# rcelha/rio-rs

Hardware: AMD Instinct MI355X
Metric: placement decisions/sec + achieved HBM GB/s, 10M objects x 1 024 nodes (higher is better)
Workload: dtype u32; 1 GPU; config 3: 10000000 objects x 1024 nodes, Zipf(1.1) load, cap 1.25x; a stream of committed ticks that starts from the cold table (all pending); objects_per_gpu=10000000, nodes=1024, parallelism=rows sharded x1

## Files before the change

### include/rio_gpu_placement_debug.h

```cpp
#ifndef RIO_GPU_PLACEMENT_DEBUG_H
#define RIO_GPU_PLACEMENT_DEBUG_H

#include "rio_gpu_placement.h"

#ifdef __cplusplus
extern "C" {
#endif

int rio_gp_debug_set_compact(rio_gp_t* h, int mode);
uint64_t rio_gp_debug_chained_scans(rio_gp_t* h);
int rio_gp_debug_set_speculate(rio_gp_t* h, int speculate);
int rio_gp_debug_set_node_index(rio_gp_t* h, uint32_t tile_rows);
int rio_gp_debug_node_index_geometry(rio_gp_t* h, const uint64_t* node_bitmap, uint32_t* out4);
void rio_gp_debug_set_scan_nt(int mode);
void rio_gp_debug_set_part_shift(int shift);
uint64_t rio_gp_debug_wave_row_lo(uint64_t n_objects, uint32_t n_nodes, uint32_t wave, uint32_t* n_waves);
int rio_gp_debug_ktrace(rio_gp_t* h, int enable, int table, uint64_t* out2048);
int rio_gp_debug_stream_probe(rio_gp_t* h, int mode, int reps, float* ms);

#ifdef __cplusplus
}
#endif
#endif
```

### rio-rs_amd/csrc/placement_kernels.h

```cpp
#pragma once
#include <hip/hip_runtime.h>
#include <stdint.h>

namespace riogp {

typedef uint32_t u32;
typedef unsigned long long u64;

constexpr u32 kNone = 0xFFFFFFFFu;
constexpr u32 kSpillMark = 0xFFFFFFFEu;
constexpr u32 kSkipMark = 0xFFFFFFFDu;
constexpr u32 kAffInactive = 0xFFFFFFFEu;
constexpr u32 kFlagReplaced = 0x10u;
constexpr u32 kNoCut = 0xFFFFFFFFu;

constexpr int kWaves = 16;
constexpr int kBlock = kWaves * 64;
constexpr int kTile = 256;
constexpr u32 kMaxBlocks = 256;
constexpr u32 kMaxSubs = 256;
constexpr int kMidBatch = 16384;
constexpr int kReqBatch = 131072;
constexpr int kSmallBatch = 256;

// ... 53 lines not shown
    u32* cutidx;
    u32* forced_bits;
    u64* rank_base;
    const u64* pending_global;
    const u64* run_if = nullptr;
    u64* RP;
    u64* R;
    u64* D;
    const u64* used_snap;
    u64* Tg = nullptr;
    DevStats* stats;
    FxRows fx;
};
constexpr u32 kFillRounds = 8;

struct PackOut {
    u32* idx;
    u32* load;
    u32* aff;
    u32* next;
    u32* wcnt;
};

struct Table {
    const u32* cur;
    const u32* load;
    const u32* aff;
    u32* next;
    const u32* pk_idx = nullptr;
    u32* real_next = nullptr;
// ... 27 lines not shown
                 hipStream_t s, hipEvent_t e0 = nullptr, hipEvent_t e1 = nullptr, const PackOut* pack = nullptr,
                 const ScanChain* chain = nullptr);
void launch_resolve(const Plan& p, const NodeTab& nt, const SolveBufs& b, u64* host_partial, hipStream_t s,
                    hipEvent_t e0 = nullptr, hipEvent_t e1 = nullptr, const PackOut* search = nullptr,
                    u64* fold_into = nullptr, u32 fold_rounds = 0, const u64* kept_from = nullptr, const u64* fold_from = nullptr);
bool inc_scan_fits(u32 m);
void launch_inc_scan(const Plan& p, u32* assign, const u32* load, const u32* aff, const NodeTab& nt, const SolveBufs& b,
                     const PackOut& pack, hipStream_t s);
Plan rebal_plan(const Plan& p);
u64 rebal_rows(u64 n);
void launch_rebal(const Plan& p, const Plan& pv, const PackOut& src, const NodeTab& nt, const PackOut& dst, const SolveBufs& b,
                  hipStream_t s);
unsigned resolve_blocks(u32 m);
void set_scan_nt(int mode);
void launch_cut_find(const Plan& p, const Table& t, const NodeTab& nt, const SolveBufs& b, bool virt, hipStream_t s,
                     bool have_cutblk);
void launch_fill(const Plan& p, const Table& t, const NodeTab& nt, const SolveBufs& b, bool virt, bool apply, bool fill,
                 int round, bool last, hipStream_t s, const PackOut* pack = nullptr);
bool fill_can_pack(u32 m);
bool cut_apply_fits(u32 m);
void launch_cut_apply(const Plan& p, const Table& t, const NodeTab& nt, const SolveBufs& b, const PackOut& pk, const PackOut& ul,
                      u64* Tg, bool pack, bool all_alive, hipStream_t s);
void launch_used_fold(u64* used, const u64* D, u32 m, u32 rounds, hipStream_t s);
#ifdef RIO_GP_LAB
int ktrace_enable(int on);
int ktrace_read(int table, u64* out );
float sync_probe(int mode, int reps, hipStream_t s);
float stream_probe(int mode, const u32* a, const u32* b, const u32* c, u32* o, u64 n, int reps, hipStream_t s,
                   hipEvent_t e0, hipEvent_t e1);
#endif

struct SmallInline { u32 a[4]; u32 b[4]; };
void launch_lookup_small(const u32* assign, u64 n_obj, const u32* idx, u32 n, u32* out, DevStats* st, hipStream_t s,
                         u32* done, u32 seq, const SmallInline* inl = nullptr);
void launch_lookup(const u32* assign, u64 n_obj, const u32* idx, u64 n, u32* out, DevStats* st, hipStream_t s,
                   u32* done = nullptr, u32 seq = 0, unsigned int* ticket = nullptr);
void launch_update(u32* assign, u64 n_obj, u32 m, const u32* idx, const u32* node, u64 n, u32* pos_scratch,
                   DevStats* st, hipStream_t s, u32* aff_life = nullptr, unsigned int* ticket = nullptr, u32* done = nullptr,
                   u32 seq = 0, u64* used = nullptr, const u32* load = nullptr);
void launch_update_small(u32* assign, const u32* idx, const u32* node, u32 n, hipStream_t s, u32* aff_life = nullptr,
                         u32* done = nullptr, u32 seq = 0, const SmallInline* inl = nullptr, u64* used = nullptr,
// ... 186 lines not shown
```

### rio-rs_amd/csrc/placement_kernels.hip

```cpp
#include "placement_kernels.h"
#include <algorithm>
#include <cstdlib>

#include <hip/hip_ext.h>

namespace riogp {


template <int CTRL>
__device__ __forceinline__ u64 dpp64(u64 v) {
    const u32 lo = (u32)__builtin_amdgcn_update_dpp(0, (int)(u32)v, CTRL, 0xf, 0xf, false);
    const u32 hi = (u32)__builtin_amdgcn_update_dpp(0, (int)(u32)(v >> 32), CTRL, 0xf, 0xf, false);
    return ((u64)hi << 32) | lo;
}
template <int CTRL>
__device__ __forceinline__ u32 dpp32(u32 v) {
    return (u32)__builtin_amdgcn_update_dpp(0, (int)v, CTRL, 0xf, 0xf, false);
}
__device__ __forceinline__ u64 shfl_up64(u64 v, int d) {
    u32 lo = __shfl_up((u32)v, d, 64), hi = __shfl_up((u32)(v >> 32), d, 64);
    return ((u64)hi << 32) | lo;
}
__device__ __forceinline__ u64 shfl_xor64(u64 v, int d) {
    u32 lo = __shfl_xor((u32)v, d, 64), hi = __shfl_xor((u32)(v >> 32), d, 64);
// ... 63 lines not shown
    wend = wave_row_lo(p, gw + 1);
    if (wend > p.n) wend = p.n;
    if (wstart > wend) wstart = wend;
}
__device__ __forceinline__ bool packed_live(const Plan& p, u64 i) {
    if (!p.wcnt) return true;
    const u64 tile = i / kTile;
    u64 gw = ((tile + 1) * p.nw - 1) / p.tiles;
    return i - wave_row_lo(p, gw) < p.wcnt[gw];
}
__device__ __forceinline__ u64 block_row_lo(const Plan& p, u32 b) { return wave_row_lo(p, (u64)b * kWaves); }
constexpr int kSmall = 128;
__device__ __forceinline__ bool bit_of(const u32* bits, u32 j) { return (bits[j >> 5] >> (j & 31)) & 1u; }

#ifdef RIO_GP_LAB
constexpr int kKtTables = 8;
__device__ u64 g_kt[kKtTables][kMaxBlocks * 8];
static int g_trace_host = 0;
#define RIOGP_KT(pl, tab, slot) do { if (threadIdx.x == 0 && (pl).trace && blockIdx.x < kMaxBlocks) g_kt[tab][(size_t)blockIdx.x * 8 + (slot)] = wall_clock64(); } while (0)
#define RIOGP_KTF(flag, tab, slot) do { if (threadIdx.x == 0 && (flag) && blockIdx.x < kMaxBlocks) g_kt[tab][(size_t)blockIdx.x * 8 + (slot)] = wall_clock64(); } while (0)
int ktrace_enable(int on) { g_trace_host = on; return 0; }
int ktrace_read(int table, u64* out) {
    if (table < 0 || table >= kKtTables) return -1;
    return (int)hipMemcpyFromSymbol(out, HIP_SYMBOL(g_kt), sizeof(u64) * kMaxBlocks * 8, sizeof(u64) * kMaxBlocks * 8 * (size_t)table);
}
static inline u32 trace_flag() { return (u32)g_trace_host; }
#else
#define RIOGP_KT(pl, tab, slot) do { } while (0)
#define RIOGP_KTF(flag, tab, slot) do { } while (0)
static inline u32 trace_flag() { return 0; }
#endif

Plan make_plan(u64 n, u32 m, u32 max_blocks) {
    Plan p;
    p.n = n;
    p.m = m;
    p.mwords = (m + 31) / 32;
    p.wcnt = nullptr;
    p.alive_dst = nullptr;
    p.trace = trace_flag();
    p.sa = 0;
    p.mark = 1;
// ... 1093 lines not shown
        r[1] += load;
    } else if (cnt) {
        atomicAdd(&stats->rejected, cnt);
        atomicAdd(&stats->load_rejected, load);
    }
}

constexpr u32 kSlotNone = 0xFFFFu;
constexpr int kCutMinSubs = 16;

__host__ __device__ __forceinline__ size_t cut_fused_fixed(u32 m, u32 mwords) {
    const u32 mr = (m + 7) & ~7u;
    return kSmall + (size_t)mr * 8 + (size_t)((mwords + 3) & ~3u) * sizeof(u32) + 2 * kWaves * sizeof(u64);
}

template <bool VIRT>
__device__ __forceinline__ void cut_search_block(unsigned char* smem, const u32 b, const u32 sel_mod, const u32 sel_rem,
                                                 const bool write_forced, const u32* __restrict__ cur,
                                                 const u32* __restrict__ load, const u32* __restrict__ aff,
                                                 const u32* __restrict__ alive_bits, const Plan& p,
                                                 const u32* __restrict__ cutblk, const u64* __restrict__ budget,
                                                 const u64* __restrict__ admpre, const u64* __restrict__ used_kept,
                                                 const u32* __restrict__ forced_bits, u32* __restrict__ cutidx,
                                                 u64* __restrict__ used_cur, const u32 tcap, u64* __restrict__ R) {
    const u32 m = p.m, mr = (m + 7) & ~7u;
    const bool sa_ = p.sa != 0;
    u32& nlocal = *reinterpret_cast<u32*>(smem);
    u64* red = reinterpret_cast<u64*>(smem + 16);
    u32* thr = reinterpret_cast<u32*>(smem + kSmall);
    unsigned short* slot = reinterpret_cast<unsigned short*>(thr + mr);
    unsigned short* node_of = slot + mr;
    u32* alv = reinterpret_cast<u32*>(node_of + mr);
    u64* rlo = reinterpret_cast<u64*>(alv + ((p.mwords + 3) & ~3u));
    u64* whi = rlo + kWaves;
    u64* T = whi + kWaves;
    const int tid = threadIdx.x, lane = tid & 63, wave = __builtin_amdgcn_readfirstlane(tid >> 6);
    if (tid == 0) { nlocal = 0; red[0] = 0; red[1] = 0; red[2] = 0; red[3] = 0; }
    const u64 gw = (u64)b * kWaves + wave;
    const u32 cb0 = cutblk[(u32)tid < m ? (u32)tid : m - 1];
// ... 36 lines not shown
        if (S > BT) S = BT;
    }
    if (S < 1) S = 1;
    const u32 Sp = (S | 1u) < 3u ? 3u : (S | 1u);
    u32 K = tcap / (Sp + 3);
    if (K < 1) K = 1;
    u64 bend = block_row_lo(p, b + 1);
    if (bend > p.n) bend = p.n;
    u32 live_tiles;
    {
        const u32 mine = lane < kWaves ? (u32)((whi[lane & (kWaves - 1)] > rlo[lane & (kWaves - 1)]
                                                     ? whi[lane & (kWaves - 1)] - rlo[lane & (kWaves - 1)] + kTile - 1 : 0) / kTile) : 0u;
        live_tiles = wave_sum32(mine);
        if (live_tiles < 1) live_tiles = 1;
    }

    for (u32 g0 = 0; g0 < nloc; g0 += K) {
        const u32 kn = nloc - g0 < K ? nloc - g0 : K;
        u64* st_bud = T + tcap - 3 * (size_t)K;
        u64* st_pre = st_bud + K;
        u64* st_rs = st_pre + K;
        for (u32 ls = tid; ls < kn; ls += kBlock) {
            st_bud[ls] = budget[node_of[g0 + ls]];
            st_pre[ls] = 0;
            st_rs[ls] = 0;
        }
        u32 rlen = BT;
        for (u32 level = 0;; ++level) {
            const u32 ptiles = (rlen + S - 1) / S;
            const u32 np = (rlen + ptiles - 1) / ptiles;
            for (u32 k = tid; k < kn * Sp; k += kBlock) T[k] = 0;
            __syncthreads();
            if (kn == 1) {
                const u32 nd0 = (u32)node_of[g0];
                const bool live0 = p.sa || bit_of(alv, nd0);
                const u32 rs0 = (u32)st_rs[0];
                for (u64 it = wstart; it < wend; it += kTile) {
                    const u32 tb = (u32)((it - bstart) / kTile);
                    u32 t = tb / ptiles;
                    if (level != 0) {
                        const u32 off = tb - rs0;
                        if (off >= rlen) continue;
                        t = off / ptiles;
                    }
                    const u64 i0 = it + (u64)lane * 4;
                    const uint4 cv = *reinterpret_cast<const uint4*>(cur + i0);
                    const uint4 av = *reinterpret_cast<const uint4*>(aff + i0);
                    const uint4 lv = *reinterpret_cast<const uint4*>(load + i0);
                    u64 sum = 0;
#define RIOGP_ROW(C, A, L, E)                                                                              \
                    {                                                                                      \
                        const bool cin = C < m;                                                            \
                        const bool kept = VIRT ? cin : (cin & bit_of(alv, cin ? C : 0u));                  \
                        const bool hit = (i0 + E < wend) & !kept & !(VIRT && C == kSkipMark) & (A == nd0) & live0; \
                        sum += hit ? (u64)L : 0ull;                                                        \
                    }
                    RIOGP_ROW(cv.x, av.x, lv.x, 0)
                    RIOGP_ROW(cv.y, av.y, lv.y, 1)
                    RIOGP_ROW(cv.z, av.z, lv.z, 2)
                    RIOGP_ROW(cv.w, av.w, lv.w, 3)
#undef RIOGP_ROW
                    sum = wave_sum(sum);
                    if (lane == 0 && sum) atomicAdd(&T[t], sum);
                }
            } else {
                uint4 cvn = make_uint4(0, 0, 0, 0), avn = cvn, lvn = cvn;
                if (wstart < wend) {
                    const u64 f0 = wstart + (u64)lane * 4;
                    cvn = *reinterpret_cast<const uint4*>(cur + f0);
                    avn = *reinterpret_cast<const uint4*>(aff + f0);
                    lvn = *reinterpret_cast<const uint4*>(load + f0);
                }
                for (u64 it = wstart; it < wend; it += kTile) {
                    const u64 i0 = it + (u64)lane * 4;
                    const uint4 cv = cvn, av = avn, lv = lvn;
                    {
                        const u64 pn = (it + kTile < wend ? it + kTile : it) + (u64)lane * 4;
                        cvn = *reinterpret_cast<const uint4*>(cur + pn);
                        avn = *reinterpret_cast<const uint4*>(aff + pn);
                        lvn = *reinterpret_cast<const uint4*>(load + pn);
                    }
                    const u32 tb = (u32)((it - bstart) / kTile);
                    const u32 t_lvl0 = tb / ptiles;
    #define RIOGP_ROW(C, A, L, E)                                                                              \
                    {                                                                                          \
                         \
                        const bool cin = C < m, ain = A < m;                                                   \
                        const u32 cx = cin ? C : 0u, ax = ain ? A : 0u;                                        \
                        const bool kept = VIRT ? cin : (cin & bit_of(alv, cx));                                \
                        const u32 ls = (u32)slot[ax] - g0;                    \
                        bool hit = (i0 + E < wend) & !kept & !(VIRT && C == kSkipMark) & ain & (sa_ | bit_of(alv, ax)) & (ls < kn); \
                        u32 t = 0;                                                                             \
                        if (level == 0) {                                                                      \
                            t = t_lvl0;   \
                        } else if (hit) {                                                                      \
                            const u32 off = tb - (u32)st_rs[ls];    \
                            hit = off < rlen;                                                                  \
                            t = off / ptiles;                                                                  \
                        }                                                                                      \
                        const u64 todo = __ballot(hit);                                                        \
                        if (__popcll(todo) >= 16) {  \
                            const int ld = __ffsll((long long)todo) - 1;                                       \
                            const u32 s0 = (u32)__shfl((int)(ls * Sp + t), ld, 64);                            \
                            const bool same = hit && ls * Sp + t == s0;                                        \
                            if (__popcll(__ballot(same)) >= 16) {                                              \
                                const u64 sum = wave_sum(same ? (u64)L : 0ull);                                \
                                if (lane == ld) atomicAdd(&T[s0], sum);                                        \
                                hit = hit && !same;                                                            \
                            }                                                                                  \
                        }                                                                                      \
                        if (hit) atomicAdd(&T[ls * Sp + t], (u64)L);                                           \
                    }
                    RIOGP_ROW(cv.x, av.x, lv.x, 0)
                    RIOGP_ROW(cv.y, av.y, lv.y, 1)
                    RIOGP_ROW(cv.z, av.z, lv.z, 2)
                    RIOGP_ROW(cv.w, av.w, lv.w, 3)
    #undef RIOGP_ROW
                }
            }
            __syncthreads();
            const u32 cost_lane = ((np + 7) / 8) * 100u;
            const u32 cost_wave = ((kn + kWaves - 1) / kWaves) * (((np + 63) / 64) * 80u + 120u);
            if (cost_lane <= cost_wave) {
                for (u32 ls = tid; ls < kn; ls += kBlock) {
                    const u64* Tj = T + (size_t)ls * Sp;
                    const u64 bud = st_bud[ls];
                    u64 acc = 0;
                    u32 tstar = np;
                    for (u32 t0 = 0; t0 < np && tstar == np; t0 += 8) {
                        u64 v[8];
#pragma unroll
                        for (int q = 0; q < 8; ++q) v[q] = t0 + q < np ? Tj[t0 + q] : 0ull;
#pragma unroll
                        for (int q = 0; q < 8; ++q) {
                            const u64 nv = acc + v[q];
// ... 140 lines not shown
                const u32 ls = base + (u32)u * kWaves;
                fetch(q[u], ls < kn ? ls : base);
            }
#pragma unroll
            for (int u = 0; u < kInFlight; ++u)
                if (base + (u32)u * kWaves < kn) run(q[u]);
        }
        __syncthreads();
    }
    if (R && tid == 0 && red[1]) atomicAdd(&R[b], (u64)0 - red[1]);
}

constexpr u32 kCutPerItem = 16;
constexpr u32 kCutMaxSlices = 64;
constexpr u32 kCutFindGrid = 256;

template <bool VIRT>
__global__ __launch_bounds__(kBlock) void k_cut_find(const u32* __restrict__ cur, const u32* __restrict__ load,
                                                     const u32* __restrict__ aff, const u32* __restrict__ alive_bits,
                                                     Plan p, const u32* __restrict__ cutblk,
                                                     const u64* __restrict__ budget, const u64* __restrict__ admpre,
                                                     const u64* __restrict__ used_kept,
                                                     const u32* __restrict__ forced_bits, u32* __restrict__ cutidx,
                                                     u64* __restrict__ used_cur, DevStats* __restrict__ stats, u32 tcap,
                                                     u64* __restrict__ R) {
    extern __shared__ __attribute__((aligned(16))) unsigned char smem[];
    __shared__ u32 cnt[kMaxBlocks];
    __shared__ unsigned short istart[kMaxBlocks + 1];
    __shared__ unsigned char nsl[kMaxBlocks];
    const int tid = threadIdx.x, lane = tid & 63;
    const u32 m = p.m, G = p.G;
    const u64 ncut = stats->n_cut;
    const u32 cb0 = cutblk[(u32)tid < m ? (u32)tid : m - 1];
    if (ncut == 0 && forced_bits == nullptr) return;
    if (forced_bits && blockIdx.x == 0)
        for (u32 j = tid; j < m; j += kBlock)
            if (bit_of(forced_bits, j)) { cutidx[j] = 0; used_cur[j] = used_kept[j]; }
    for (u32 k = tid; k < kMaxBlocks; k += kBlock) cnt[k] = 0;
    __syncthreads();
    for (u32 j = tid; j < m; j += kBlock) {
        const u32 cb = j == (u32)tid ? cb0 : cutblk[j];
        if (cb < G && !(forced_bits && bit_of(forced_bits, j))) atomicAdd(&cnt[cb], 1u);
    }
    __syncthreads();
    if (tid < 64) {
        u32 c[4], tot = 0;
#pragma unroll
        for (int q = 0; q < 4; ++q) {
            const u32 bq = (u32)tid * 4 + q;
// ... 3 lines not shown
            c[q] = sl;
            tot += sl;
        }
        const u64 inc = wave_incl_scan((u64)tot, lane);
        u32 ex = (u32)inc - tot;
#pragma unroll
        for (int q = 0; q < 4; ++q) {
            istart[tid * 4 + q] = (unsigned short)ex;
            nsl[tid * 4 + q] = (unsigned char)c[q];
            ex += c[q];
        }
        if (tid == 63) istart[kMaxBlocks] = (unsigned short)inc;
    }
    __syncthreads();
    const u32 items = istart[kMaxBlocks];
    for (u32 item = blockIdx.x; item < items; item += gridDim.x) {
        u32 lo = 0, hi = kMaxBlocks;
        while (hi - lo > 1) {
            const u32 mid = lo + ((hi - lo) >> 1);
            if (istart[mid] <= item) lo = mid; else hi = mid;
        }
        __syncthreads();
        cut_search_block<VIRT>(smem, lo, nsl[lo], item - istart[lo], false, cur, load, aff, alive_bits, p, cutblk, budget,
                               admpre, used_kept, forced_bits, cutidx, used_cur, tcap, R);
    }
}

__device__ u64 block_excl_scan_1024(u64 v, bool saturating, u64* lds_part , u64* total) {
    const int tid = threadIdx.x, lane = tid & 63, wave = tid >> 6;
    const u64 inc = saturating ? wave_incl_scan_sat(v, lane) : wave_incl_scan(v, lane);
    if (lane == 63) lds_part[wave] = inc;
    __syncthreads();
    u64 base = 0, tot = 0;
    for (int w = 0; w < kWaves; ++w) {
        const u64 x = lds_part[w];
        if (w < wave) base = saturating ? sat_add(base, x) : base + x;
        tot = saturating ? sat_add(tot, x) : tot + x;
    }
    __syncthreads();
    if (total) *total = tot;
// ... 2950 lines not shown
        else hipLaunchKernelGGL(k_resolve<false>, dim3(grid), dim3(256), 0, s, a);
    }
}

static size_t cut_find_lds(const Plan& p, u32* tcap_out) {
    const size_t fixed = cut_fused_fixed(p.m, p.mwords);
    size_t slots = (150 * 1024 - fixed) / sizeof(u64);
    const size_t most = (size_t)p.m * 259;
    if (slots > most) slots = most;
    if (slots < 64) slots = 64;
    *tcap_out = (u32)slots;
    return fixed + slots * sizeof(u64);
}

void launch_cut_find(const Plan& p, const Table& t, const NodeTab& nt, const SolveBufs& b, bool virt, hipStream_t s,
                     bool have_cutblk) {
    const unsigned gcb = (p.m + kCbNodes - 1) / kCbNodes;
    if (!have_cutblk)
        hipLaunchKernelGGL(k_cutblk, dim3(gcb ? gcb : 1), dim3(256), 0, s, b.H, p, nt.cap, nt.alive_bits, b.used_kept,
                           b.claim_tot, b.cutblk, b.budget, b.admpre, b.stats);
    u32 tcap = 0;
    const size_t ldsf = cut_find_lds(p, &tcap);
    u64* R = have_cutblk ? b.R : nullptr;
    if (virt)
        hipLaunchKernelGGL(k_cut_find<true>, dim3(kCutFindGrid), dim3(kBlock), ldsf, s, t.cur, t.load, t.aff, nt.alive_bits, p,
                           b.cutblk, b.budget, b.admpre, b.used_kept, b.forced_bits, b.cutidx, b.used_cur, b.stats, tcap, R);
    else
        hipLaunchKernelGGL(k_cut_find<false>, dim3(kCutFindGrid), dim3(kBlock), ldsf, s, t.cur, t.load, t.aff, nt.alive_bits, p,
                           b.cutblk, b.budget, b.admpre, b.used_kept, b.forced_bits, b.cutidx, b.used_cur, b.stats, tcap, R);
}

static size_t fill_lds_bytes(u32 m, u32 mwords, bool pack) { return fill_lds_off_x(m) + fill_lds_x(m, mwords, pack) + 16; }
bool fill_can_pack(u32 m) { return fill_lds_bytes(m, (m + 31) / 32, true) <= (size_t)160 * 1024; }

void launch_fill(const Plan& p, const Table& t, const NodeTab& nt, const SolveBufs& b, bool virt, bool apply, bool fill,
                 int round, bool last, hipStream_t s, const PackOut* pack) {
    const int in = (apply ? 0 : (round & 1)), out = fill ? (in ^ 1) : 0;
    FillArgs a;
    a.cur = t.cur; a.load = t.load; a.aff = t.aff; a.next = t.next;
    a.alive_bits = nt.alive_bits;
    a.p = p;
    a.cutidx = b.cutidx; a.forced_bits = b.forced_bits;
    a.cap = nt.cap; a.round = (u32)round;
    if (b.D) { a.Uread = b.used_cur; a.D = b.D; a.Uadd = b.D + (size_t)round * p.m; }
// ... 1527 lines not shown
```

### rio-rs_amd/csrc/rio_gp_capi.hip

```cpp
#include <hip/hip_runtime.h>
#include <dlfcn.h>

#include <cstdio>
#include <cstdlib>
#include <cstring>
#include <chrono>
#include <algorithm>
#include <atomic>
#include <mutex>
#include <string>
#include <vector>

#include "../../include/rio_gpu_placement.h"
#ifdef RIO_GP_LAB
#include "../../include/rio_gpu_placement_debug.h"
#endif
#include "placement_kernels.h"

using namespace riogp;

namespace {

thread_local std::string g_create_error;
struct RioGpNcclId { char internal[128]; };
// ... 200 lines not shown
    u32* chain_flags = nullptr;
    u32 *h_chain_err = nullptr, *d_chain_err = nullptr;
    u32 chain_seq = 0, chain_prev = 0, chain_pos = 0;
    hipEvent_t ev_run = nullptr;
    u64 overlap_min_rows = (u64)1 << 18;
    hipEvent_t ev_join = nullptr;
    u64* used_ring = nullptr;
    size_t used_slot_words = 0;
    u32 used_base = 0;
    int chain_diag = 0;
    bool chain_ok = false;
    u64 chain_total = 0;
    int chain_mode = 0;
    int cutapply_mode = 0;
    int spec_mode = 0;
    int part_mode = 0;
    u32* h_cs = nullptr;
    u32* d_cs = nullptr;
    size_t cs_words = 0;
    u64* cs_cnt = nullptr;
    unsigned int* cs_ticket = nullptr;
    u32* h_small = nullptr;
    u32* d_small = nullptr;
    u64 wait_seq = 1;
    u32* h_mid = nullptr;
    u32* d_mid = nullptr;
    unsigned int* mid_ticket = nullptr;
    u32* h_req = nullptr;
    u32* d_req = nullptr;
    u32* pp_bad = nullptr;
// ... 250 lines not shown
    if (!virt && !f.resolve_searches && !p.wcnt && f.cut_apply) {
        launch_cut_apply(p, t, nt, h->sb, h->pk, h->pk2, h->Tg, cutpack, h->all_alive, h->stream);
        if (cutpack) {
            Plan pp = p;
            pp.wcnt = h->pk.wcnt;
            Table vt{h->pos , h->pk.load, h->pk.aff, h->pk.next};
            vt.pk_idx = h->pk.idx;
            vt.real_next = t.next;
            vt.none_prewritten = true;
            for (u32 r = 0; r < h->rounds; ++r) launch_fill(pp, vt, nt, h->sb, true, false, true, (int)r, r + 1 == h->rounds, h->stream);
        } else {
            for (u32 r = 0; r < h->rounds; ++r) launch_fill(p, t, nt, h->sb, false, false, true, (int)r, r + 1 == h->rounds, h->stream);
        }
        return;
    }
    if (!f.resolve_searches) launch_cut_find(p, t, nt, h->sb, virt, h->stream, true);
    launch_fill(p, t, nt, h->sb, virt, true, true, 0, h->rounds == 1, h->stream, cutpack ? &h->pk : nullptr);
    if (cutpack) {
        Plan pp = p;
        pp.wcnt = h->pk.wcnt;
        Table vt{h->pos , h->pk.load, h->pk.aff, h->pk.next};
        vt.pk_idx = h->pk.idx;
        vt.real_next = t.next;
        vt.none_prewritten = true;
        for (u32 r = 1; r < h->rounds; ++r) launch_fill(pp, vt, nt, h->sb, true, false, true, (int)r, r + 1 == h->rounds, h->stream);
        return;
    }
    for (u32 r = 1; r < h->rounds; ++r) launch_fill(p, t, nt, h->sb, virt, false, true, (int)r, r + 1 == h->rounds, h->stream);
}

PendingSolve enqueue_scan_resolve(rio_gp* h, const SolveForm& f, const Table& t, const NodeTab& nt, u64* host_rows) {
// ... 382 lines not shown
#define A(ptr, cnt) if ((rc = dalloc(h, &(ptr), (cnt))) != RIO_GP_OK) return bail(rc)
    A(h->assign[0], R); A(h->assign[1], R); A(h->load, R); A(h->aff, R); A(h->pos, R2);
    h->used_slot_words = (h->chain_ok ? (size_t)kChainReps : 1) * M;
    A(h->cap, M); A(h->used_ring, kUsedRing * h->used_slot_words); A(h->alive_bits, (M + 31) / 32 + 4); A(h->dead_bits, (M + 31) / 32 + 4);
    A(h->alive_bytes, M);
    A(h->sb.H, (size_t)((M + 7) / 8) * kMaxBlocks * 16); A(h->sb.blkstat, (size_t)kMaxBlocks * 4);
    A(h->sb.partial, (size_t)resolve_blocks((u32)M) * 8 + 8);
    A(h->sb.wsp_sum[0], W); A(h->sb.wsp_sum[1], W); A(h->sb.wsp_cnt[0], W); A(h->sb.wsp_cnt[1], W);
    A(h->sb.bsp_sum[0], (size_t)kMaxBlocks); A(h->sb.bsp_sum[1], (size_t)kMaxBlocks); A(h->sb.bsp_cnt[0], (size_t)kMaxBlocks); A(h->sb.bsp_cnt[1], (size_t)kMaxBlocks);
    A(h->sb.used_kept, M); A(h->sb.claim_tot, M); A(h->sb.cutblk, M); A(h->sb.budget, M);
    A(h->sb.admpre, M); A(h->sb.cutidx, M); A(h->dstats, 1); A(h->fx_dev, (size_t)kMaxBlocks * 8);
    A(h->sb.R, (size_t)kMaxBlocks); A(h->sb.RP, (size_t)kMaxBlocks * resolve_blocks((u32)M)); A(h->D, (size_t)kFillRounds * M);
    A(h->pk.idx, R); A(h->pk.load, R); A(h->pk.aff, R); A(h->pk.next, R); A(h->pk.wcnt, W);
    A(h->pk2.idx, R2); A(h->pk2.load, R2); A(h->pk2.aff, R2); A(h->pk2.next, R2); A(h->pk2.wcnt, W);
    A(h->Tg, M * kWaves);
    A(h->chain_flags, W);
    A(h->sh_lkept, M); A(h->sh_lclaim, M); A(h->sh_lcur, M); A(h->sh_lcutblk, M); A(h->sh_lcutidx, M);
    A(h->sh_gprev, M); A(h->sh_gfinal, M); A(h->sh_rank_base, 2); A(h->sh_verdict, 8); A(h->sh_forced, (M + 31) / 32 + 4);
#undef A
    h->used.init(h, h->used_ring);
    h->sb.used_cur = h->used_ring + h->used_slot_words;
    h->sb.stats = h->dstats;
    if (hipHostMalloc(reinterpret_cast<void**>(&h->h_stats), sizeof(DevStats) * kRing, hipHostMallocMapped) !=
        hipSuccess) {
        h->err = "hipHostMalloc failed";
        return bail(RIO_GP_ENOMEM);
    }
    if (hipHostMalloc(reinterpret_cast<void**>(&h->h_chain_err), 64, hipHostMallocMapped) != hipSuccess ||
        hipHostGetDevicePointer(reinterpret_cast<void**>(&h->d_chain_err), h->h_chain_err, 0) != hipSuccess) {
        h->err = "hipHostMalloc(chain error word) failed";
// ... 58 lines not shown
        h->err = "request staging allocation failed";
        return bail(RIO_GP_ENOMEM);
    }
    h->allocs.push_back(h->pp_stage);
    launch_fill_u32(h->assign[0], R, kNone, h->stream);
    launch_fill_u32(h->assign[1], R, kNone, h->stream);
    launch_fill_u32(h->pos, R2, kNone, h->stream);
    launch_fill_u32(h->load, R, 0, h->stream);
    launch_fill_u32(h->aff, R, kNone, h->stream);
    (void)hipMemsetAsync(h->used_ring, 0, kUsedRing * h->used_slot_words * sizeof(u64), h->stream);
    (void)hipMemsetAsync(h->alive_bits, 0, ((M + 31) / 32 + 4) * sizeof(u32), h->stream);
    (void)hipMemsetAsync(h->dstats, 0, sizeof(DevStats), h->stream);
    (void)hipMemsetAsync(h->D, 0, (size_t)kFillRounds * M * sizeof(u64), h->stream);
    (void)hipMemsetAsync(h->sb.R, 0, (size_t)kMaxBlocks * sizeof(u64), h->stream);
    (void)hipMemsetAsync(h->chain_flags, 0, W * sizeof(u32), h->stream);
    if (hipStreamSynchronize(h->stream) != hipSuccess || hipGetLastError() != hipSuccess) {
        h->err = "initial fill failed (no gfx950 code object loaded?)";
        return bail(RIO_GP_EUPSTREAM);
    }
    *out = h;
    return RIO_GP_OK;
}

void rio_gp_destroy(rio_gp_t* h) {
    if (!h) return;
    (void)hipSetDevice(h->device);
    if (h->stream) (void)hipStreamSynchronize(h->stream);
    if (h->own_stream && h->own_stream != h->stream) (void)hipStreamSynchronize(h->own_stream);
    if (h->scan2) (void)hipStreamSynchronize(h->scan2);
    shard_comm_free(h);
// ... 2224 lines not shown
        return rc;
    }
    if (!h->sc) return fail(h, RIO_GP_EINVAL, "rio_gp_shard_exchange: call rio_gp_shard_comm_init first");
    const int rc = h->sc->api.AllGather(d_in, d_out, (size_t)words, kNcclUint64, h->sc->comm, h->stream);
    if (rc != 0) return fail(h, RIO_GP_EUPSTREAM, "ncclAllGather failed");
    return RIO_GP_OK;
}

#ifdef RIO_GP_LAB
void rio_gp_debug_set_scan_nt(int mode) { set_scan_nt(mode); }
void rio_gp_debug_set_part_shift(int shift) { set_part_shift(shift); }
uint64_t rio_gp_debug_wave_row_lo(uint64_t n_objects, uint32_t n_nodes, uint32_t wave, uint32_t* n_waves) {
    return plan_wave_row_lo(n_objects, n_nodes, wave, n_waves);
}

int rio_gp_debug_set_compact(rio_gp_t* h, int mode) {
    if (!h || mode < 0 || mode >= 8192 || (mode & 2048) || (mode & 15) > 2 || ((mode >> 5) & 3) == 3) return RIO_GP_EINVAL;
    Locked g(h);
    h->part_mode = (mode & 16) ? 2 : 0;
    h->cutpack_mode = (mode >> 5) & 3;
    h->compact_mode = mode & 15;
    h->inc_mode = (mode >> 7) & 3;
    if (h->inc_mode == 3) h->inc_mode = 0;
    h->cutapply_mode = (mode >> 9) & 3;
    if (h->cutapply_mode == 3) h->cutapply_mode = 0;
    h->chain_mode = (mode & 4096) ? 2 : 0;
    return RIO_GP_OK;
}

uint64_t rio_gp_debug_chained_scans(rio_gp_t* h) {
// ... 82 lines not shown
```

### rio-rs_amd/rio_gp.py

```python
import ctypes as C
import os
import subprocess

import numpy as np

_DIR = os.path.dirname(os.path.abspath(__file__))
LIB_PATH = os.path.join(_DIR, "librio_gp.so")
NONE = 0xFFFFFFFF
CAP_INF = 0xFFFFFFFFFFFFFFFF
AFF_INACTIVE = 0xFFFFFFFE
CFG_ROW_LIFECYCLE = 1
CFG_REF_SELF_ASSIGN = 2
OP_CFG_NO_HOST_SHADOW = 8
OP_CFG_LIVE_FIRST_TOUCH = 4
FLAG_LOCAL, FLAG_REDIRECT, FLAG_PLACED, FLAG_SPILLED, FLAG_UNPLACED = range(5)
FLAG_REPLACED = 0x10
FLAG_MASK = 0x0F
CHANGES_PEEK = 1
NODE_GONE = 0xFFFFFFFC
OK, EINVAL, EUPSTREAM, ENODEV, ENOMEM, ERANGE, EAGAIN = range(7)
ABI_VERSION = 2

LAB_PATH = os.path.join(_DIR, "librio_gp_lab.so")
SOURCES = [os.path.join(_DIR, "csrc", f) for f in ("placement_kernels.hip", "rio_gp_capi.hip", "gpu_object_placement.cpp")]
# ... 169 lines not shown
        L.rio_gp_remap_nodes.argtypes = [_vp, C.c_uint32, _vp, C.POINTER(C.c_uint64)]
        if lab:
            L.rio_gp_debug_set_scan_nt.argtypes = [C.c_int]
            L.rio_gp_debug_set_scan_nt.restype = None
            L.rio_gp_debug_set_part_shift.argtypes = [C.c_int]
            L.rio_gp_debug_set_part_shift.restype = None
            L.rio_gp_debug_stream_probe.argtypes = [_vp, C.c_int, C.c_int, C.POINTER(C.c_float)]
            L.rio_gp_debug_set_compact.argtypes = [_vp, C.c_int]
            L.rio_gp_debug_set_speculate.argtypes = [_vp, C.c_int]
            L.rio_gp_debug_chained_scans.argtypes = [_vp]
            L.rio_gp_debug_chained_scans.restype = C.c_uint64
            L.rio_gp_debug_ktrace.argtypes = [_vp, C.c_int, C.c_int, C.POINTER(C.c_uint64)]
            L.rio_gp_debug_wave_row_lo.argtypes = [C.c_uint64, C.c_uint32, C.c_uint32, C.POINTER(C.c_uint32)]
            L.rio_gp_debug_wave_row_lo.restype = C.c_uint64
            L.rio_gp_debug_set_node_index.argtypes = [_vp, C.c_uint32]
            L.rio_gp_debug_node_index_geometry.argtypes = [_vp, _vp, _vp]
        L.rio_gp_timer_begin.argtypes = [_vp]
        L.rio_gp_timer_stop.argtypes = [_vp]
        L.rio_gp_timer_end.argtypes = [_vp, C.POINTER(C.c_float)]
        _libs[lab] = L
    return _libs[lab]


def _ptr(a):
    return None if a is None else a.ctypes.data_as(_vp)


def _u32(a):
    return None if a is None else np.ascontiguousarray(a, dtype=np.uint32)

# ... 355 lines not shown
        return float(ms.value)

    def ktrace(self, enable=True, table=None):
        self._need_lab()
        out = (C.c_uint64 * 2048)() if table is not None else None
        self._chk(self._L.rio_gp_debug_ktrace(self._h, 1 if enable else 0, 0 if table is None else table, out))
        return np.ctypeslib.as_array(out).reshape(256, 8).copy() if table is not None else None

    def set_compact(self, mode, partitioned_crud=True, cut_pack="auto", inc="auto", cut_apply="auto", chain=True):
        self._need_lab()
        modes = {"auto": 0, "always": 1, "never": 2}
        incs = {"auto": 0, "always": 1, "never": 2}
        self._chk(self._L.rio_gp_debug_set_compact(self._h, modes.get(mode, mode) | (0 if partitioned_crud else 16) |
                                                   (modes.get(cut_pack, cut_pack) << 5) | (incs.get(inc, inc) << 7) |
                                                   (modes.get(cut_apply, cut_apply) << 9) | (0 if chain else 4096)))

    def chained_scans(self):
        self._need_lab()
        return int(self._L.rio_gp_debug_chained_scans(self._h))

    def set_node_index(self, tile_rows=0):
        self._need_lab()
        self._chk(self._L.rio_gp_debug_set_node_index(self._h, int(tile_rows)))

    def node_index_geometry(self, nodes=None):
        self._need_lab()
        out = np.zeros(4, np.uint32)
        self._chk(self._L.rio_gp_debug_node_index_geometry(self._h, _ptr(self._node_bitmap(nodes)), _ptr(out)))
        return tuple(int(x) for x in out)

# ... 309 lines not shown
```

Measured before the change: 427.8 billion decisions/s.

## Split cut-find search items across multiple blocks with ticketed partial-sum merge

```diff
diff --git a/include/rio_gpu_placement_debug.h b/include/rio_gpu_placement_debug.h
--- a/include/rio_gpu_placement_debug.h
+++ b/include/rio_gpu_placement_debug.h
@@ -16,6 +16,8 @@
 void rio_gp_debug_set_part_shift(int shift);
 uint64_t rio_gp_debug_wave_row_lo(uint64_t n_objects, uint32_t n_nodes, uint32_t wave, uint32_t* n_waves);
 int rio_gp_debug_ktrace(rio_gp_t* h, int enable, int table, uint64_t* out2048);
+void rio_gp_debug_set_cut_split(int max_items);
+int rio_gp_debug_cut_split_counts(rio_gp_t* h, uint64_t* out2);
 int rio_gp_debug_stream_probe(rio_gp_t* h, int mode, int reps, float* ms);
 
 #ifdef __cplusplus
diff --git a/rio-rs_amd/csrc/placement_kernels.h b/rio-rs_amd/csrc/placement_kernels.h
--- a/rio-rs_amd/csrc/placement_kernels.h
+++ b/rio-rs_amd/csrc/placement_kernels.h
@@ -91,6 +91,16 @@
 };
 constexpr u32 kFillRounds = 8;
 
+constexpr u32 kCutSplitUnits = 16;
+constexpr u32 kCutSplitSlots = 16;
+constexpr u32 kCutSplitStride = 256;
+constexpr u32 kCutSplitMaxItems = 64;
+struct CutSplit {
+    u64* sum = nullptr;
+    u32* ticket = nullptr;
+    u32 max_items = 0;
+};
+
 struct PackOut {
     u32* idx;
     u32* load;
@@ -148,7 +158,7 @@
 unsigned resolve_blocks(u32 m);
 void set_scan_nt(int mode);
 void launch_cut_find(const Plan& p, const Table& t, const NodeTab& nt, const SolveBufs& b, bool virt, hipStream_t s,
-                     bool have_cutblk);
+                     bool have_cutblk, const CutSplit* split = nullptr);
 void launch_fill(const Plan& p, const Table& t, const NodeTab& nt, const SolveBufs& b, bool virt, bool apply, bool fill,
                  int round, bool last, hipStream_t s, const PackOut* pack = nullptr);
 bool fill_can_pack(u32 m);
@@ -159,6 +169,8 @@
 #ifdef RIO_GP_LAB
 int ktrace_enable(int on);
 int ktrace_read(int table, u64* out );
+void set_cut_split(int max_items);
+int cut_split_counts(u64* out2);
 float sync_probe(int mode, int reps, hipStream_t s);
 float stream_probe(int mode, const u32* a, const u32* b, const u32* c, u32* o, u64 n, int reps, hipStream_t s,
                    hipEvent_t e0, hipEvent_t e1);
diff --git a/rio-rs_amd/csrc/placement_kernels.hip b/rio-rs_amd/csrc/placement_kernels.hip
--- a/rio-rs_amd/csrc/placement_kernels.hip
+++ b/rio-rs_amd/csrc/placement_kernels.hip
@@ -101,7 +101,7 @@
 __device__ __forceinline__ bool bit_of(const u32* bits, u32 j) { return (bits[j >> 5] >> (j & 31)) & 1u; }
 
 #ifdef RIO_GP_LAB
-constexpr int kKtTables = 8;
+constexpr int kKtTables = 9;
 __device__ u64 g_kt[kKtTables][kMaxBlocks * 8];
 static int g_trace_host = 0;
 #define RIOGP_KT(pl, tab, slot) do { if (threadIdx.x == 0 && (pl).trace && blockIdx.x < kMaxBlocks) g_kt[tab][(size_t)blockIdx.x * 8 + (slot)] = wall_clock64(); } while (0)
@@ -112,7 +112,11 @@
     return (int)hipMemcpyFromSymbol(out, HIP_SYMBOL(g_kt), sizeof(u64) * kMaxBlocks * 8, sizeof(u64) * kMaxBlocks * 8 * (size_t)table);
 }
 static inline u32 trace_flag() { return (u32)g_trace_host; }
+__device__ u64 g_cf_split[2];
+#define RIOGP_CF_COUNT(slot, v) atomicAdd(&g_cf_split[slot], (u64)(v))
+int cut_split_counts(u64* out2) { return (int)hipMemcpyFromSymbol(out2, HIP_SYMBOL(g_cf_split), sizeof(u64) * 2); }
 #else
+#define RIOGP_CF_COUNT(slot, v) do { } while (0)
 #define RIOGP_KT(pl, tab, slot) do { } while (0)
 #define RIOGP_KTF(flag, tab, slot) do { } while (0)
 static inline u32 trace_flag() { return 0; }
@@ -1236,7 +1240,7 @@
     return kSmall + (size_t)mr * 8 + (size_t)((mwords + 3) & ~3u) * sizeof(u32) + 2 * kWaves * sizeof(u64);
 }
 
-template <bool VIRT>
+template <bool VIRT, bool SPLIT = false>
 __device__ __forceinline__ void cut_search_block(unsigned char* smem, const u32 b, const u32 sel_mod, const u32 sel_rem,
                                                  const bool write_forced, const u32* __restrict__ cur,
                                                  const u32* __restrict__ load, const u32* __restrict__ aff,
@@ -1244,7 +1248,9 @@
                                                  const u32* __restrict__ cutblk, const u64* __restrict__ budget,
                                                  const u64* __restrict__ admpre, const u64* __restrict__ used_kept,
                                                  const u32* __restrict__ forced_bits, u32* __restrict__ cutidx,
-                                                 u64* __restrict__ used_cur, const u32 tcap, u64* __restrict__ R) {
+                                                 u64* __restrict__ used_cur, const u32 tcap, u64* __restrict__ R,
+                                                 const u32 sp_units = 0, const u32 sp_item = 0, const u32 sp_chunk = 0,
+                                                 u64* sp_sum = nullptr, u32* sp_ticket = nullptr) {
     const u32 m = p.m, mr = (m + 7) & ~7u;
     const bool sa_ = p.sa != 0;
     u32& nlocal = *reinterpret_cast<u32*>(smem);
@@ -1311,6 +1317,26 @@
         live_tiles = wave_sum32(mine);
         if (live_tiles < 1) live_tiles = 1;
     }
+    u64 it_lo = wstart, it_hi = wend, it_step = kTile;
+    bool presplit = false;
+    u32 ch_t0 = 0, ch_t1 = 0;
+    if (SPLIT && sp_units) {
+        if (nloc == 0) return;
+        const u32 pt0 = (BT + S - 1) / S, np0 = (BT + pt0 - 1) / pt0;
+        if (nloc <= kCutSplitSlots && nloc <= K && np0 <= kCutSplitStride) {
+            presplit = true;
+            const u32 cp = (np0 + sp_units - 1) / sp_units;
+            ch_t0 = sp_chunk * cp < np0 ? sp_chunk * cp : np0;
+            ch_t1 = ch_t0 + cp < np0 ? ch_t0 + cp : np0;
+            it_lo = bstart + ((u64)ch_t0 * pt0 + (u32)wave) * kTile;
+            it_hi = bstart + (u64)ch_t1 * pt0 * kTile;
+            if (it_hi > bend) it_hi = bend;
+            it_step = (u64)kWaves * kTile;
+        } else if (sp_chunk != 0) {
+            return;
+        }
+        RIOGP_KT(p, 8, 1);
+    }
 
     for (u32 g0 = 0; g0 < nloc; g0 += K) {
         const u32 kn = nloc - g0 < K ? nloc - g0 : K;
@@ -1332,7 +1358,7 @@
                 const u32 nd0 = (u32)node_of[g0];
                 const bool live0 = p.sa || bit_of(alv, nd0);
                 const u32 rs0 = (u32)st_rs[0];
-                for (u64 it = wstart; it < wend; it += kTile) {
+                for (u64 it = it_lo; it < it_hi; it += it_step) {
                     const u32 tb = (u32)((it - bstart) / kTile);
                     u32 t = tb / ptiles;
                     if (level != 0) {
@@ -1349,7 +1375,7 @@
                     {                                                                                      \
                         const bool cin = C < m;                                                            \
                         const bool kept = VIRT ? cin : (cin & bit_of(alv, cin ? C : 0u));                  \
-                        const bool hit = (i0 + E < wend) & !kept & !(VIRT && C == kSkipMark) & (A == nd0) & live0; \
+                        const bool hit = (i0 + E < it_hi) & !kept & !(VIRT && C == kSkipMark) & (A == nd0) & live0; \
                         sum += hit ? (u64)L : 0ull;                                                        \
                     }
                     RIOGP_ROW(cv.x, av.x, lv.x, 0)
@@ -1362,17 +1388,17 @@
                 }
             } else {
                 uint4 cvn = make_uint4(0, 0, 0, 0), avn = cvn, lvn = cvn;
-                if (wstart < wend) {
-                    const u64 f0 = wstart + (u64)lane * 4;
+                if (it_lo < it_hi) {
+                    const u64 f0 = it_lo + (u64)lane * 4;
                     cvn = *reinterpret_cast<const uint4*>(cur + f0);
                     avn = *reinterpret_cast<const uint4*>(aff + f0);
                     lvn = *reinterpret_cast<const uint4*>(load + f0);
                 }
-                for (u64 it = wstart; it < wend; it += kTile) {
+                for (u64 it = it_lo; it < it_hi; it += it_step) {
                     const u64 i0 = it + (u64)lane * 4;
                     const uint4 cv = cvn, av = avn, lv = lvn;
                     {
-                        const u64 pn = (it + kTile < wend ? it + kTile : it) + (u64)lane * 4;
+                        const u64 pn = (it + it_step < it_hi ? it + it_step : it) + (u64)lane * 4;
                         cvn = *reinterpret_cast<const uint4*>(cur + pn);
                         avn = *reinterpret_cast<const uint4*>(aff + pn);
                         lvn = *reinterpret_cast<const uint4*>(load + pn);
@@ -1386,7 +1412,7 @@
                         const u32 cx = cin ? C : 0u, ax = ain ? A : 0u;                                        \
                         const bool kept = VIRT ? cin : (cin & bit_of(alv, cx));                                \
                         const u32 ls = (u32)slot[ax] - g0;                    \
-                        bool hit = (i0 + E < wend) & !kept & !(VIRT && C == kSkipMark) & ain & (sa_ | bit_of(alv, ax)) & (ls < kn); \
+                        bool hit = (i0 + E < it_hi) & !kept & !(VIRT && C == kSkipMark) & ain & (sa_ | bit_of(alv, ax)) & (ls < kn); \
                         u32 t = 0;                                                                             \
                         if (level == 0) {                                                                      \
                             t = t_lvl0;   \
@@ -1416,6 +1442,43 @@
                 }
             }
             __syncthreads();
+            if (SPLIT && presplit && level == 0) {
+                RIOGP_KT(p, 8, 2);
+                u64* const base = sp_sum + (size_t)sp_item * kCutSplitSlots * kCutSplitStride;
+                auto rank_of = [&](u32 ls) -> u32 {
+                    const u32 me = node_of[ls];
+                    u32 d = 0;
+                    for (u32 q = 0; q < nloc; ++q) d += (u32)node_of[q] < me;
+                    return d;
+                };
+                const u32 ct = ch_t1 - ch_t0;
+                for (u32 k = tid; k < kn * ct; k += kBlock) {
+                    const u32 ls = k / ct, t = ch_t0 + k % ct;
+                    __hip_atomic_store(base + (size_t)rank_of(ls) * kCutSplitStride + t, T[(size_t)ls * Sp + t], __ATOMIC_RELAXED,
+                                       __HIP_MEMORY_SCOPE_AGENT);
+                }
+                asm volatile("s_waitcnt vmcnt(0)" ::: "memory");
+                __syncthreads();
+                if (tid == 0) {
+                    const u32 tk = __hip_atomic_fetch_add(sp_ticket + sp_item, 1u, __ATOMIC_RELAXED, __HIP_MEMORY_SCOPE_AGENT);
+                    red[2] = tk == sp_units - 1 ? 1ull : 0ull;
+                }
+                __syncthreads();
+                RIOGP_KT(p, 8, 3);
+                if (red[2] == 0) return;
+                for (u32 k = tid; k < kn * np; k += kBlock) {
+                    const u32 ls = k / np, t = k % np;
+                    T[(size_t)ls * Sp + t] = __hip_atomic_load(base + (size_t)rank_of(ls) * kCutSplitStride + t, __ATOMIC_RELAXED,
+                                                               __HIP_MEMORY_SCOPE_AGENT);
+                }
+                if (tid == 0) {
+                    __hip_atomic_store(sp_ticket + sp_item, 0u, __ATOMIC_RELAXED, __HIP_MEMORY_SCOPE_AGENT);
+                    RIOGP_CF_COUNT(0, 1);
+                }
+                it_lo = wstart; it_hi = wend; it_step = kTile;
+                __syncthreads();
+                RIOGP_KT(p, 8, 4);
+            }
             const u32 cost_lane = ((np + 7) / 8) * 100u;
             const u32 cost_wave = ((kn + kWaves - 1) / kWaves) * (((np + 63) / 64) * 80u + 120u);
             if (cost_lane <= cost_wave) {
@@ -1586,6 +1649,10 @@
 constexpr u32 kCutPerItem = 16;
 constexpr u32 kCutMaxSlices = 64;
 constexpr u32 kCutFindGrid = 256;
+static int g_cut_split_items = 32;
+#ifdef RIO_GP_LAB
+void set_cut_split(int max_items) { g_cut_split_items = max_items < 0 ? 32 : max_items > (int)kCutSplitMaxItems ? (int)kCutSplitMaxItems : max_items; }
+#endif
 
 template <bool VIRT>
 __global__ __launch_bounds__(kBlock) void k_cut_find(const u32* __restrict__ cur, const u32* __restrict__ load,
@@ -1595,7 +1662,7 @@
                                                      const u64* __restrict__ used_kept,
                                                      const u32* __restrict__ forced_bits, u32* __restrict__ cutidx,
                                                      u64* __restrict__ used_cur, DevStats* __restrict__ stats, u32 tcap,
-                                                     u64* __restrict__ R) {
+                                                     u64* __restrict__ R, CutSplit cs) {
     extern __shared__ __attribute__((aligned(16))) unsigned char smem[];
     __shared__ u32 cnt[kMaxBlocks];
     __shared__ unsigned short istart[kMaxBlocks + 1];
@@ -1605,6 +1672,7 @@
     const u64 ncut = stats->n_cut;
     const u32 cb0 = cutblk[(u32)tid < m ? (u32)tid : m - 1];
     if (ncut == 0 && forced_bits == nullptr) return;
+    RIOGP_KT(p, 8, 0);
     if (forced_bits && blockIdx.x == 0)
         for (u32 j = tid; j < m; j += kBlock)
             if (bit_of(forced_bits, j)) { cutidx[j] = 0; used_cur[j] = used_kept[j]; }
@@ -1638,16 +1706,30 @@
     }
     __syncthreads();
     const u32 items = istart[kMaxBlocks];
-    for (u32 item = blockIdx.x; item < items; item += gridDim.x) {
+    bool split = !VIRT && cs.sum != nullptr && forced_bits == nullptr && p.wcnt == nullptr && items != 0 && items <= cs.max_items;
+    u32 per = 1;
+    if (split) {
+        const u32 need = (p.subs * (p.sub / kTile) + kWaves - 1) / kWaves;
+        per = gridDim.x / items;
+        if (per > need) per = need < 2 ? 2 : need;
+        if (per > kCutSplitUnits) per = kCutSplitUnits;
+        if (per < 2) split = false, per = 1;
+    }
+
+    if (split && blockIdx.x == 0 && tid == 0) RIOGP_CF_COUNT(1, items * per);
+    for (u32 unit = blockIdx.x; unit < items * per; unit += gridDim.x) {
+        const u32 item = unit / per;
         u32 lo = 0, hi = kMaxBlocks;
         while (hi - lo > 1) {
             const u32 mid = lo + ((hi - lo) >> 1);
             if (istart[mid] <= item) lo = mid; else hi = mid;
         }
         __syncthreads();
-        cut_search_block<VIRT>(smem, lo, nsl[lo], item - istart[lo], false, cur, load, aff, alive_bits, p, cutblk, budget,
-                               admpre, used_kept, forced_bits, cutidx, used_cur, tcap, R);
-    }
+        cut_search_block<VIRT, !VIRT>(smem, lo, nsl[lo], item - istart[lo], false, cur, load, aff, alive_bits, p, cutblk, budget,
+                                      admpre, used_kept, forced_bits, cutidx, used_cur, tcap, R, split ? per : 0u, item, unit % per, cs.sum,
+                                      cs.ticket);
+    }
+    RIOGP_KT(p, 8, 7);
 }
 
 __device__ u64 block_excl_scan_1024(u64 v, bool saturating, u64* lds_part , u64* total) {
@@ -4628,7 +4710,7 @@
 }
 
 void launch_cut_find(const Plan& p, const Table& t, const NodeTab& nt, const SolveBufs& b, bool virt, hipStream_t s,
-                     bool have_cutblk) {
+                     bool have_cutblk, const CutSplit* split) {
     const unsigned gcb = (p.m + kCbNodes - 1) / kCbNodes;
     if (!have_cutblk)
         hipLaunchKernelGGL(k_cutblk, dim3(gcb ? gcb : 1), dim3(256), 0, s, b.H, p, nt.cap, nt.alive_bits, b.used_kept,
@@ -4636,12 +4718,17 @@
     u32 tcap = 0;
     const size_t ldsf = cut_find_lds(p, &tcap);
     u64* R = have_cutblk ? b.R : nullptr;
+    CutSplit cs;
+    if (split && !virt) {
+        cs = *split;
+        cs.max_items = (u32)g_cut_split_items < cs.max_items ? (u32)g_cut_split_items : cs.max_items;
+    }
     if (virt)
         hipLaunchKernelGGL(k_cut_find<true>, dim3(kCutFindGrid), dim3(kBlock), ldsf, s, t.cur, t.load, t.aff, nt.alive_bits, p,
-                           b.cutblk, b.budget, b.admpre, b.used_kept, b.forced_bits, b.cutidx, b.used_cur, b.stats, tcap, R);
+                           b.cutblk, b.budget, b.admpre, b.used_kept, b.forced_bits, b.cutidx, b.used_cur, b.stats, tcap, R, cs);
     else
         hipLaunchKernelGGL(k_cut_find<false>, dim3(kCutFindGrid), dim3(kBlock), ldsf, s, t.cur, t.load, t.aff, nt.alive_bits, p,
-                           b.cutblk, b.budget, b.admpre, b.used_kept, b.forced_bits, b.cutidx, b.used_cur, b.stats, tcap, R);
+                           b.cutblk, b.budget, b.admpre, b.used_kept, b.forced_bits, b.cutidx, b.used_cur, b.stats, tcap, R, cs);
 }
 
 static size_t fill_lds_bytes(u32 m, u32 mwords, bool pack) { return fill_lds_off_x(m) + fill_lds_x(m, mwords, pack) + 16; }
diff --git a/rio-rs_amd/csrc/rio_gp_capi.hip b/rio-rs_amd/csrc/rio_gp_capi.hip
--- a/rio-rs_amd/csrc/rio_gp_capi.hip
+++ b/rio-rs_amd/csrc/rio_gp_capi.hip
@@ -238,6 +238,7 @@
     int chain_mode = 0;
     int cutapply_mode = 0;
     int spec_mode = 0;
+    CutSplit cf;
     int part_mode = 0;
     u32* h_cs = nullptr;
     u32* d_cs = nullptr;
@@ -518,7 +519,8 @@
         }
         return;
     }
-    if (!f.resolve_searches) launch_cut_find(p, t, nt, h->sb, virt, h->stream, true);
+    if (!f.resolve_searches)
+        launch_cut_find(p, t, nt, h->sb, virt, h->stream, true, !virt && !p.wcnt && !h->sb.forced_bits ? &h->cf : nullptr);
     launch_fill(p, t, nt, h->sb, virt, true, true, 0, h->rounds == 1, h->stream, cutpack ? &h->pk : nullptr);
     if (cutpack) {
         Plan pp = p;
@@ -931,6 +933,8 @@
     A(h->pk.idx, R); A(h->pk.load, R); A(h->pk.aff, R); A(h->pk.next, R); A(h->pk.wcnt, W);
     A(h->pk2.idx, R2); A(h->pk2.load, R2); A(h->pk2.aff, R2); A(h->pk2.next, R2); A(h->pk2.wcnt, W);
     A(h->Tg, M * kWaves);
+    A(h->cf.sum, (size_t)kCutSplitMaxItems * kCutSplitSlots * kCutSplitStride); A(h->cf.ticket, (size_t)kCutSplitMaxItems);
+    h->cf.max_items = kCutSplitMaxItems;
     A(h->chain_flags, W);
     A(h->sh_lkept, M); A(h->sh_lclaim, M); A(h->sh_lcur, M); A(h->sh_lcutblk, M); A(h->sh_lcutidx, M);
     A(h->sh_gprev, M); A(h->sh_gfinal, M); A(h->sh_rank_base, 2); A(h->sh_verdict, 8); A(h->sh_forced, (M + 31) / 32 + 4);
@@ -1019,6 +1023,8 @@
     (void)hipMemsetAsync(h->D, 0, (size_t)kFillRounds * M * sizeof(u64), h->stream);
     (void)hipMemsetAsync(h->sb.R, 0, (size_t)kMaxBlocks * sizeof(u64), h->stream);
     (void)hipMemsetAsync(h->chain_flags, 0, W * sizeof(u32), h->stream);
+    (void)hipMemsetAsync(h->cf.sum, 0, (size_t)kCutSplitMaxItems * kCutSplitSlots * kCutSplitStride * sizeof(u64), h->stream);
+    (void)hipMemsetAsync(h->cf.ticket, 0, (size_t)kCutSplitMaxItems * sizeof(u32), h->stream);
     if (hipStreamSynchronize(h->stream) != hipSuccess || hipGetLastError() != hipSuccess) {
         h->err = "initial fill failed (no gfx950 code object loaded?)";
         return bail(RIO_GP_EUPSTREAM);
@@ -3273,6 +3279,16 @@
     return plan_wave_row_lo(n_objects, n_nodes, wave, n_waves);
 }
 
+void rio_gp_debug_set_cut_split(int max_items) { set_cut_split(max_items); }
+int rio_gp_debug_cut_split_counts(rio_gp_t* h, uint64_t* out2) {
+    if (!h || !out2) return RIO_GP_EINVAL;
+    Locked g(h);
+    HIPCHK(h, hipSetDevice(h->device));
+    HIPCHK(h, hipStreamSynchronize(h->stream));
+    if (cut_split_counts(reinterpret_cast<u64*>(out2)) != 0) return fail(h, RIO_GP_EUPSTREAM, "cut split counters read failed");
+    return RIO_GP_OK;
+}
+
 int rio_gp_debug_set_compact(rio_gp_t* h, int mode) {
     if (!h || mode < 0 || mode >= 8192 || (mode & 2048) || (mode & 15) > 2 || ((mode >> 5) & 3) == 3) return RIO_GP_EINVAL;
     Locked g(h);
diff --git a/rio-rs_amd/rio_gp.py b/rio-rs_amd/rio_gp.py
--- a/rio-rs_amd/rio_gp.py
+++ b/rio-rs_amd/rio_gp.py
@@ -207,6 +207,9 @@
             L.rio_gp_debug_wave_row_lo.argtypes = [C.c_uint64, C.c_uint32, C.c_uint32, C.POINTER(C.c_uint32)]
             L.rio_gp_debug_wave_row_lo.restype = C.c_uint64
             L.rio_gp_debug_set_node_index.argtypes = [_vp, C.c_uint32]
+            L.rio_gp_debug_set_cut_split.argtypes = [C.c_int]
+            L.rio_gp_debug_set_cut_split.restype = None
+            L.rio_gp_debug_cut_split_counts.argtypes = [_vp, C.POINTER(C.c_uint64)]
             L.rio_gp_debug_node_index_geometry.argtypes = [_vp, _vp, _vp]
         L.rio_gp_timer_begin.argtypes = [_vp]
         L.rio_gp_timer_stop.argtypes = [_vp]
@@ -592,6 +595,16 @@
         self._chk(self._L.rio_gp_debug_set_compact(self._h, modes.get(mode, mode) | (0 if partitioned_crud else 16) |
                                                    (modes.get(cut_pack, cut_pack) << 5) | (incs.get(inc, inc) << 7) |
                                                    (modes.get(cut_apply, cut_apply) << 9) | (0 if chain else 4096)))
+
+    def set_cut_split(self, max_items=None):
+        self._need_lab()
+        self._L.rio_gp_debug_set_cut_split(-1 if max_items is None else int(max_items))
+
+    def cut_split_counts(self):
+        self._need_lab()
+        out = (C.c_uint64 * 2)()
+        self._chk(self._L.rio_gp_debug_cut_split_counts(self._h, out))
+        return int(out[0]), int(out[1])
 
     def chained_scans(self):
         self._need_lab()
```

New measurement: 427.7 billion decisions/s (median of 2 runs). No clear change (-0.0%).
